# PANXIONG-CN/TEC-MoLLM

Hardware: AMD Instinct MI355X
Metric: train samples/sec (higher is better)
Workload: dtype f32; 1 GPU; BASELINE configs[1]: B=8/GPU, L_in=48, L_out=12, N=2911, F=10 (d_emb=12), 3 GPT-2 blocks, full fwd+bwd+AdamW, fp32, GATv2 per_timestep, dropout on (p=0.1); global_batch=8, parallelism=dp1, data_feed=fixed, launch=eager

## Files before the change

### include/tecmollm.h

```cpp
#ifndef TECMOLLM_H
#define TECMOLLM_H

#include <stdint.h>

#ifdef __cplusplus
extern "C" {
#endif

#define TECM_OK 0
#define TECM_E_ARG (-1)
#define TECM_E_ALIGN (-2)
#define TECM_E_LAUNCH (-3)
#define TECM_E_LDS (-4)

#define TECM_ABI_VERSION 21
int tecm_abi_version(void);
const char* tecm_last_error(void);

typedef struct TecmWin {
  int32_t enabled;
  int32_t N;
  int32_t Lin, Lout;
  int32_t stride_t;
  int32_t taps;
// ... 132 lines not shown
                       void* stream);

#define TECM_ATT_OUT_BF16 1
#define TECM_ATT_QKV_BF16 2
#define TECM_ATT_DCTX_BF16 4
int tecm_attention_fwd(const float* qkv, void* ctx, int32_t io_bf16, int32_t B, int32_t T, int32_t N, int32_t heads,
                       int32_t D, const TecmDrop* prob_drop, void* stream);
int tecm_attention_bwd(const float* qkv, const float* dctx, void* dqkv, int32_t io_bf16, int32_t B, int32_t T, int32_t N,
                       int32_t heads, int32_t D, const TecmDrop* prob_drop, void* stream);

int tecm_colsum(const float* in, int64_t ld, int64_t outer, int64_t inner, int32_t nseg, int32_t C,
                float* out, int64_t ldo, int32_t accumulate, float scale, const TecmDrop* in_drop,
                float* workspace , void* stream);
int tecm_colsum_twin(const float* in, int64_t ld, int64_t outer, int64_t inner, int32_t nseg, int32_t C,
                     float* out, int64_t ldo, int32_t accumulate, float scale, const TecmDrop* in_drop,
                     float* workspace, void* twin_bf16, int64_t ld_twin, void* stream);

int tecm_colsum_batch(const float* const* in, float* const* out, int32_t nbuf, int64_t ld, int64_t rows, int32_t C,
                      float* workspace , void* stream);

int tecm_huber_fwd_bwd(const float* pred, const float* target, float* dpred, float* loss_out,
                       int64_t n, float delta, float grad_scale, float* workspace ,
                       void* stream);

int tecm_conv_weight_pack(const float* w, float* fwd_pack, float* bwd_pack, int32_t Cout, int32_t Cin,
                          int32_t k, void* stream);
int tecm_conv_weight_unpack(const float* dpack, float* dw, int32_t Cout, int32_t Cin, int32_t k,
                            void* stream);

typedef struct TecmConvDx {
  const void* dy;
  const void* wpack;
  float* dinp;
  int32_t B, Lc, N, Cout, ld_in, _pad;
} TecmConvDx;
int tecm_conv_dx_pack(const float* w3, const float* w5, const float* w7, void* wpack, int32_t Cout, int32_t Cin,
                      int32_t ld_in, void* stream);
int tecm_conv_dx_bf16(const TecmConvDx* p, void* stream);
typedef struct TecmConvFwd {
  const void* inp;
  const void* wpack;
  const float* bias;
  float* y;
  int32_t B, Lc, N, Cout, ld_in, y_bf16;
  float* stats;
  float eps;
  int32_t _pad;
} TecmConvFwd;
int tecm_conv_fwd_pack(const float* w3, const float* w5, const float* w7, void* wpack, int32_t Cout, int32_t Cin,
                       int32_t ld_in, void* stream);
int tecm_conv_fwd_bf16(const TecmConvFwd* p, void* stream);
int tecm_conv_fwd_pack_f32(const float* w3, const float* w5, const float* w7, float* wpack, int32_t Cout, int32_t Cin,
                           int32_t ld_in, void* stream);
int tecm_conv_fwd_f32(const TecmConvFwd* p, void* stream);
int tecm_conv_dx_pack_f32(const float* w3, const float* w5, const float* w7, float* wpack, int32_t Cout, int32_t Cin,
                          int32_t ld_in, void* stream);
int tecm_conv_dx_f32(const TecmConvDx* p, void* stream);
int tecm_conv_fwd_supported(int32_t Lc, int32_t Cout, int32_t ld_in, int32_t f32);
int tecm_conv_dx_supported(int32_t Lc, int32_t Cout, int32_t ld_in, int32_t f32);
int tecm_conv_fwd_stats_supported(int32_t Lc);

typedef struct TecmConvDw {
  const void* inp;
  const void* dy;
  float* workspace;
  float* dw3;
  float* dw5;
// ... 103 lines not shown
```

### tec-mollm_amd/csrc/conv_seq.hip

```cpp
#include "common.h"
#include <type_traits>

typedef float f32x16 __attribute__((ext_vector_type(16)));
typedef __bf16 bf16x8 __attribute__((ext_vector_type(8)));
typedef unsigned int u32x4 __attribute__((ext_vector_type(4)));
typedef float f32x4 __attribute__((ext_vector_type(4)));

namespace tecm_convseq {

#ifndef CDX_ABLATE
#define CDX_ABLATE 0
#endif

constexpr int NB = 4;
constexpr int NTH = 256;
constexpr int MAXT = 6;

__host__ __device__ __forceinline__ int seg_nact(int d) {
  const int a = d < 3 ? 3 - d : d - 3;
  return a <= 1 ? 3 : (a == 2 ? 2 : 1);
}

struct Args {
  const void* dy;
// ... 129 lines not shown
#pragma unroll
        for (int gq = 0; gq < 4; ++gq) {
          const int ci = 32 * c + 8 * gq + 4 * h;
          if (ci < a.ld_in)
            *reinterpret_cast<float4*>(orow + ci) = make_float4(v[4 * gq], v[4 * gq + 1], v[4 * gq + 2], v[4 * gq + 3]);
        }
      }
    }
  }
}

template <int NCI>
__global__ __launch_bounds__(NTH, 2) void conv_dx_seq_kernel(const Args a) {
  extern __shared__ __attribute__((aligned(16))) unsigned char lds[];
  const int tid = threadIdx.x, lane = tid & 63;
  const int wave = __builtin_amdgcn_readfirstlane(tid >> 6);
  const Tile t = decode_tile(a, blockIdx.x);
  {
    constexpr int SB = 12;
    const int total = t.rows * a.cpr;
    for (int q0 = 0; q0 * NTH < ((CDX_ABLATE & 1) ? 0 : total); q0 += SB) {
      u32x4 v[SB];
      stage_load<SB>(a, t, q0, v);
      stage_store<SB>(a, t, q0, v, lds);
    }
    if (tid < a.pitch / 16) *reinterpret_cast<uint4*>(lds + a.zero_off + tid * 16) = make_uint4(0u, 0u, 0u, 0u);
  }
  __syncthreads();
  tile_compute<NCI>(a, t, lds, wave, lane, false);
}

constexpr int NTH32 = 512;

template <int NCI>
__global__ __launch_bounds__(NTH32, 2) void conv_dx_seq_f32_kernel(const Args a) {
  extern __shared__ __attribute__((aligned(16))) unsigned char lds[];
  const int tid = threadIdx.x, lane = tid & 63;
  const int wave = __builtin_amdgcn_readfirstlane(tid >> 6);
  const int r = lane & 31, h = lane >> 5;
  const Tile t = decode_tile(a, blockIdx.x);
  {
    constexpr int SB = 10;
    const int total = t.rows * a.cpr;
    for (int q0 = 0; q0 * NTH32 < total; q0 += SB) {
      u32x4 v[SB];
      stage_load<SB>(a, t, q0, v);
      stage_store<SB>(a, t, q0, v, lds);
    }
    if (tid < a.pitch / 16) *reinterpret_cast<uint4*>(lds + a.zero_off + tid * 16) = make_uint4(0u, 0u, 0u, 0u);
  }
  __syncthreads();

  const int spc = a.Cout / 8;
  const int KS = 15 * spc;
  const int s_beg = wave * (KS / 8), s_end = s_beg + KS / 8;
  int d = 0, sd = s_beg;
  while (sd >= seg_nact(d) * spc) {
    sd -= seg_nact(d) * spc;
    ++d;
  }
  const int ntt = t.tc >> 3;
  f32x16 acc[MAXT];
#pragma unroll
  for (int i = 0; i < MAXT; ++i)
#pragma unroll
    for (int e = 0; e < 16; ++e) acc[i][e] = 0.f;
  const int tl0 = r >> 2;
  constexpr int WD = 3;
  const f32x4* wp = reinterpret_cast<const f32x4*>(a.wpack) + (int64_t)s_beg * NCI * 64 + lane;
  f32x4 wf[WD][NCI];
#pragma unroll
  for (int u = 0; u < WD; ++u)
#pragma unroll
    for (int c = 0; c < NCI; ++c) wf[u][c] = wp[(u * NCI + c) * 64];
  for (int s0 = s_beg; s0 < s_end; s0 += WD) {
#pragma unroll
    for (int u = 0; u < WD; ++u) {
      const int delta = d - 3;
      const int colb = ((3 - seg_nact(d)) * a.Cout + sd * 8 + 4 * h) * 4;
      const int rbase = (t.t0 - t.ts_lo + delta) * 4 + r;
#pragma unroll
      for (int i = 0; i < MAXT / NCI; ++i) {
        if (i < ntt) {
          const int ts = t.t0 + 8 * i + tl0 + delta;
          const bool ok = ts >= 0 && ts < a.Lc;
          const int off = ok ? (rbase + 32 * i) * a.pitch + colb : a.zero_off + 16 * h;
          const f32x4 df = *reinterpret_cast<const f32x4*>(lds + off);
#pragma unroll
          for (int j = 0; j < 4; ++j)
#pragma unroll
            for (int c = 0; c < NCI; ++c)
              acc[i * NCI + c] = __builtin_amdgcn_mfma_f32_32x32x2f32(wf[u][c][j], df[j], acc[i * NCI + c], 0, 0, 0);
        }
      }
      if (s0 + u + WD < s_end) {
#pragma unroll
        for (int c = 0; c < NCI; ++c) wf[u][c] = wp[((u + WD) * NCI + c) * 64];
      }
      if (++sd == seg_nact(d) * spc) {
        sd = 0;
        ++d;
      }
    }
    wp += WD * NCI * 64;
  }
  __syncthreads();

  float* part = reinterpret_cast<float*>(lds);
  const int NT = ntt * NCI;
  if (wave >= 4) {
#pragma unroll
    for (int T = 0; T < MAXT; ++T)
      if (T < NT)
#pragma unroll
        for (int e = 0; e < 16; ++e) part[(((wave - 4) * NT + T) * 16 + e) * 64 + lane] = acc[T][e];
  }
  __syncthreads();
  if (wave < 4) {
#pragma unroll
    for (int T = 0; T < MAXT; ++T)
      if (T < NT)
#pragma unroll
        for (int e = 0; e < 16; ++e) acc[T][e] += part[((wave * NT + T) * 16 + e) * 64 + lane];
  }
  __syncthreads();
  if (wave < 4) {
#pragma unroll
    for (int T = 0; T < MAXT; ++T) {
      if (T < NT && (T & 3) != wave) {
        const int slot = (wave - (T & 3) - 1) & 3;
#pragma unroll
        for (int e = 0; e < 16; ++e) part[((T * 3 + slot) * 16 + e) * 64 + lane] = acc[T][e];
      }
    }
  }
  __syncthreads();
  if (wave < 4) {
#pragma unroll
    for (int T = 0; T < MAXT; ++T) {
      if (T < NT && (T & 3) == wave) {
        f32x16 v = acc[T];
#pragma unroll
        for (int slot = 0; slot < 3; ++slot)
#pragma unroll
          for (int e = 0; e < 16; ++e) v[e] += part[((T * 3 + slot) * 16 + e) * 64 + lane];
        const int i = T / NCI, c = T % NCI;
        const int tt = t.t0 + 8 * i + tl0, n = t.n0 + (r & 3);
        if (n < a.N) {
          float* orow = a.dinp + (((int64_t)t.b * a.Lc + tt) * a.N + n) * a.ld_in;
#pragma unroll
          for (int gq = 0; gq < 4; ++gq) {
            const int ci = 32 * c + 8 * gq + 4 * h;
            if (ci < a.ld_in)
              *reinterpret_cast<float4*>(orow + ci) = make_float4(v[4 * gq], v[4 * gq + 1], v[4 * gq + 2], v[4 * gq + 3]);
          }
        }
      }
    }
  }
}

__global__ __launch_bounds__(256) void conv_dx_pack_f32_kernel(const float* __restrict__ w3, const float* __restrict__ w5,
                                                               const float* __restrict__ w7, float* __restrict__ wpack,
                                                               int Cout, int Cin, int NCI) {
  const int total = 15 * Cout * NCI * 32;
  for (int i = blockIdx.x * 256 + threadIdx.x; i < total; i += gridDim.x * 256) {
    const int j = i & 3, lane = (i >> 2) & 63;
    const int sc = i >> 8, c = sc % NCI, s = sc / NCI;
    int k = 8 * s + 4 * (lane >> 5) + j;
    const int ci = 32 * c + (lane & 31);
    int d = 0;
    while (k >= seg_nact(d) * Cout) {
      k -= seg_nact(d) * Cout;
      ++d;
    }
    const int col = (3 - seg_nact(d)) * Cout + k;
    const int jj = col / Cout, co = col - jj * Cout;
    const int kj = 3 + 2 * jj, tau = (kj - 1) / 2 - (d - 3);
    const float* w = jj == 0 ? w3 : (jj == 1 ? w5 : w7);
    float v = 0.f;
    if (ci < Cin && tau >= 0 && tau < kj) v = w[((int64_t)co * Cin + ci) * kj + tau];
    wpack[i] = v;
  }
}

__global__ __launch_bounds__(256) void conv_dx_pack_kernel(const float* __restrict__ w3, const float* __restrict__ w5,
                                                           const float* __restrict__ w7, __bf16* __restrict__ wpack,
                                                           int Cout, int Cin, int NCI) {
  const int KTOT = 15 * Cout;
  const int total = KTOT * NCI * 32;
  for (int i = blockIdx.x * 256 + threadIdx.x; i < total; i += gridDim.x * 256) {
// ... 228 lines not shown
      if (i < ntt) {
#pragma unroll
        for (int e = 0; e < 16; ++e) {
          const int n = e & 3;
          if (n0 + n < a.N) yb[(8 * i + 2 * (e >> 2)) * tstride + n * CT] = acc[i][e] + bv;
        }
      }
    }
  }
  CFW_STAMP(8);
  if (a.stats) {
    __syncthreads();
    if (tid < 3 * NB) {
      const int jb = tid / NB, n = tid % NB;
      const float ucnt = (float)(32 * tc);
      float cnt = 0.f, mean = 0.f, m2 = 0.f;
      for (int w = 0; w < 4; ++w)
        for (int q = 0; q < 3; ++q)
          if (xst[w][q][0] == (float)jb) {
            const float tot = cnt + ucnt, fr = ucnt / tot, dl = xst[w][q][1 + n] - mean;
            m2 += xst[w][q][1 + NB + n] + dl * dl * cnt * fr;
            mean += dl * fr;
            cnt = tot;
          }
      if (n0 + n < a.N) {
        float* st = a.stats + (((int64_t)b * a.N + n0 + n) * 3 + jb) * 2;
        st[0] = mean;
        st[1] = 1.0f / sqrtf(m2 / cnt + a.eps);
      }
    }
  }
}

__global__ __launch_bounds__(NTH, 2) void conv_fwd_seq_f32_kernel(const FArgs a) {
  extern __shared__ __attribute__((aligned(16))) unsigned char lds[];
  const int tid = threadIdx.x, lane = tid & 63;
  const int wave = __builtin_amdgcn_readfirstlane(tid >> 6);
  const int r = lane & 31, h = lane >> 5;
  int tile = blockIdx.x;
  const int nbk = tile % a.nblk;
  tile /= a.nblk;
  const int chunk = tile % a.nchunk, b = tile / a.nchunk;
  const int n0 = nbk * NB, t0 = chunk * a.TC;
  const int tc = min(a.TC, a.Lc - t0);
  const int steps = tc + 7;
  const int CT = 3 * a.Cout;
  {
    const int cpr = a.ld_in / 4;
    const int total = steps * NB * cpr;
    const float* src = static_cast<const float*>(a.inp);
    for (int idx = tid; idx < total; idx += NTH) {
      const int row = idx / cpr, ch = idx - row * cpr;
      const int ts = t0 - 3 + (row >> 2);
      const int ng = min(n0 + (row & 3), a.N - 1);
      u32x4 v = {0u, 0u, 0u, 0u};
      if (ts >= 0 && ts < a.Lc)
        v = *reinterpret_cast<const u32x4*>(src + (((int64_t)b * a.Lc + ts) * a.N + ng) * a.ld_in + ch * 4);
      *reinterpret_cast<u32x4*>(lds + row * a.pitch + ch * 16) = v;
    }
  }
  __syncthreads();

  const int ntt = tc >> 3;
  const int cpt = a.ld_in / 4;
  const unsigned cpt_magic = (unsigned)((65536 + cpt - 1) / cpt);
#pragma unroll 1
  for (int ui = 0; ui < 3; ++ui) {
    const int u = (int)((a.assign >> (12 * wave + 4 * ui)) & 15ull);
    if (u == 15) break;
    const int j = u / a.nb32, kb = u - j * a.nb32;
    const int pad = j + 1, col0 = j * a.Cout + 32 * kb;
    const int st3 = 3 * a.ld_in / 8, st5 = 5 * a.ld_in / 8, st7 = 7 * a.ld_in / 8;
    const int nsteps = j == 0 ? st3 : (j == 1 ? st5 : st7);
    const int woff = (j == 0 ? 0 : (j == 1 ? st3 : st3 + st5)) * a.nb32 + kb * nsteps;
    f32x16 acc[MAXT];
#pragma unroll
    for (int i = 0; i < MAXT; ++i)
#pragma unroll
      for (int e = 0; e < 16; ++e) acc[i][e] = 0.f;
    const f32x4* wp = reinterpret_cast<const f32x4*>(a.wpack) + (int64_t)woff * 64 + lane;
    auto kloop = [&](auto ntc) {
      constexpr int NTT = decltype(ntc)::value;
      auto rd = [&](int s, f32x4 (&df)[NTT]) {
        const int q = 2 * s + h;
        const int tap = (int)((q * cpt_magic) >> 16), c4 = q - tap * cpt;
        const int off0 = ((tap - pad + 3) * 4 + r) * a.pitch + c4 * 16;
#pragma unroll
        for (int i = 0; i < NTT; ++i) df[i] = *reinterpret_cast<const f32x4*>(lds + off0 + 32 * i * a.pitch);
      };
      f32x4 wq[CFW_PD32], df[NTT];
#pragma unroll
      for (int p_ = 0; p_ < CFW_PD32; ++p_) wq[p_] = wp[min(p_, nsteps - 1) * 64];
      rd(0, df);
      for (int s = 0; s < nsteps; ++s) {
        const int sn = min(s + 1, nsteps - 1);
        const f32x4 wn = wp[min(s + CFW_PD32, nsteps - 1) * 64];
        f32x4 dn[NTT];
        rd(sn, dn);
#pragma unroll
        for (int jj = 0; jj < 4; ++jj)
#pragma unroll
          for (int i = 0; i < NTT; ++i) acc[i] = __builtin_amdgcn_mfma_f32_32x32x2f32(df[i][jj], wq[0][jj], acc[i], 0, 0, 0);
#pragma unroll
        for (int p_ = 0; p_ + 1 < CFW_PD32; ++p_) wq[p_] = wq[p_ + 1];
        wq[CFW_PD32 - 1] = wn;
#pragma unroll
        for (int i = 0; i < NTT; ++i) df[i] = dn[i];
      }
    };
    switch (ntt) {
      case 1: kloop(std::integral_constant<int, 1>{}); break;
      case 2: kloop(std::integral_constant<int, 2>{}); break;
      case 3: kloop(std::integral_constant<int, 3>{}); break;
      case 4: kloop(std::integral_constant<int, 4>{}); break;
      case 5: kloop(std::integral_constant<int, 5>{}); break;
      default: kloop(std::integral_constant<int, MAXT>{}); break;
    }
    const float bv = a.bias[col0 + r];
    float* yb = a.y + (((int64_t)b * a.Lc + t0 + h) * a.N + n0) * CT + col0 + r;
    const int tstride = a.N * CT;
#pragma unroll
    for (int i = 0; i < MAXT; ++i) {
      if (i < ntt) {
#pragma unroll
        for (int e = 0; e < 16; ++e) {
          const int n = e & 3;
          if (n0 + n < a.N) yb[(8 * i + 2 * (e >> 2)) * tstride + n * CT] = acc[i][e] + bv;
        }
      }
    }
  }
}

__global__ __launch_bounds__(256) void conv_fwd_pack_f32_kernel(const float* __restrict__ w3, const float* __restrict__ w5,
                                                                const float* __restrict__ w7, float* __restrict__ wpack,
                                                                int Cout, int Cin, int ld_in) {
  const int nblk = Cout / 32;
  int steps[3], base[3], tot = 0;
  for (int j = 0; j < 3; ++j) {
    steps[j] = (3 + 2 * j) * ld_in / 8;
    base[j] = tot;
    tot += steps[j] * nblk;
  }
  const int total = tot * 256;
  for (int i = blockIdx.x * 256 + threadIdx.x; i < total; i += gridDim.x * 256) {
    const int jj = i & 3, lane = (i >> 2) & 63, f = i >> 8;
    int j = 2;
    if (f < base[1]) j = 0; else if (f < base[2]) j = 1;
    const int fl = f - base[j], blk = fl / steps[j], s = fl - blk * steps[j];
    const int k = 8 * s + 4 * (lane >> 5) + jj;
    const int tap = k / ld_in, ci = k - tap * ld_in, kj = 3 + 2 * j;
    const float* w = j == 0 ? w3 : (j == 1 ? w5 : w7);
    float v = 0.f;
    if (tap < kj && ci < Cin) v = w[((int64_t)(32 * blk + (lane & 31)) * Cin + ci) * kj + tap];
    wpack[i] = v;
  }
}

__global__ __launch_bounds__(256) void conv_fwd_pack_kernel(const float* __restrict__ w3, const float* __restrict__ w5,
                                                            const float* __restrict__ w7, __bf16* __restrict__ wpack,
                                                            int Cout, int Cin, int ld_in) {
  const int nblk = Cout / 32;
  int steps[3], base[3], tot = 0;
// ... 133 lines not shown
  return TECM_OK;
}

struct ConvDxPlan { int TC, zero_off, row_bytes, pitch, NCI; size_t lds; };
static ConvDxPlan conv_dx_plan(int Lc, int Cout, int ld_in, bool f32) {
  using namespace tecm_convseq;
  ConvDxPlan q;
  q.NCI = (ld_in + 31) / 32;
  q.row_bytes = 3 * Cout * (f32 ? 4 : 2);
  q.pitch = q.row_bytes + 16;
  int TC = 8 * (MAXT / q.NCI);
  if (TC > Lc) TC = Lc;
  auto img_steps = [&](int tc) { return tc + 6 < Lc ? tc + 6 : Lc; };
  auto zero_of = [&](int tc) {
    const size_t img = (size_t)img_steps(tc) * NB * q.pitch;
    const size_t xch = (size_t)(tc / 8) * q.NCI * (f32 ? 4 : 3) * 16 * 64 * 4;
    return img > xch ? img : xch;
  };
  while (TC > 8 && zero_of(TC) + q.pitch > 160 * 1024) TC -= 8;
  q.TC = TC;
  q.zero_off = (int)zero_of(TC);
  q.lds = zero_of(TC) + q.pitch;
  return q;
}

extern "C" int tecm_conv_dx_supported(int32_t Lc, int32_t Cout, int32_t ld_in, int32_t f32) {
  if (Lc <= 0 || Lc % 8 != 0 || Cout <= 0 || Cout % 64 != 0 || ld_in <= 0 || ld_in % 4 != 0 || ld_in > 64) return 0;
  return conv_dx_plan(Lc, Cout, ld_in, f32 != 0).lds <= 160 * 1024 ? 1 : 0;
}

static int conv_dx_launch(const TecmConvDx* p, void* stream, bool f32, const char* who) {
  using namespace tecm_convseq;
  TECM_REQUIRE(p && p->dy && p->wpack && p->dinp, TECM_E_ARG, "%s: null pointer", who);
  TECM_REQUIRE(p->B > 0 && p->Lc > 0 && p->N > 0, TECM_E_ARG, "%s: bad shape", who);
  TECM_REQUIRE(p->Cout % 64 == 0 && p->Cout > 0 && p->ld_in % 4 == 0 && p->ld_in > 0 && p->ld_in <= 64, TECM_E_ARG,
               "%s: Cout must be a multiple of 64 and ld_in a multiple of 4 up to 64", who);
  TECM_REQUIRE(p->Lc % 8 == 0, TECM_E_ARG, "%s: the sequence length must be a multiple of 8", who);
  TECM_REQUIRE(tecm_aligned(p->dy, 16) && tecm_aligned(p->wpack, 16) && tecm_aligned(p->dinp, 16), TECM_E_ALIGN,
               "%s: 16-byte aligned pointers", who);
  Args a;
  a.dy = p->dy;
  a.wpack = p->wpack;
  a.dinp = p->dinp;
  a.B = p->B; a.Lc = p->Lc; a.N = p->N; a.Cout = p->Cout; a.ld_in = p->ld_in;
  const ConvDxPlan q = conv_dx_plan(p->Lc, p->Cout, p->ld_in, f32);
  a.NCI = q.NCI;
  a.row_bytes = q.row_bytes;
  a.cpr = a.row_bytes / 16;
  a.pitch = q.pitch;
  const size_t lds = q.lds;
  TECM_REQUIRE(lds <= 160 * 1024, TECM_E_LDS, "%s: %d channels need %zu B of LDS per tile", who, 3 * p->Cout, lds);
  const int TC = q.TC;
  a.TC = TC;
  a.zero_off = q.zero_off;
  a.nchunk = (p->Lc + TC - 1) / TC;
  a.nblk = (p->N + NB - 1) / NB;
  const int64_t tiles = (int64_t)p->B * a.nchunk * a.nblk;
  TECM_REQUIRE(tiles < ((int64_t)1 << 31), TECM_E_ARG, "%s: too many tiles", who);
  const void* fn = f32 ? (a.NCI == 1 ? reinterpret_cast<const void*>(&conv_dx_seq_f32_kernel<1>)
                                     : reinterpret_cast<const void*>(&conv_dx_seq_f32_kernel<2>))
                       : (a.NCI == 1 ? reinterpret_cast<const void*>(&conv_dx_seq_kernel<1>)
                                     : reinterpret_cast<const void*>(&conv_dx_seq_kernel<2>));
  TECM_REQUIRE(hipFuncSetAttribute(fn, hipFuncAttributeMaxDynamicSharedMemorySize, 160 * 1024) == hipSuccess, TECM_E_LAUNCH,
               "%s: hipFuncSetAttribute(MaxDynamicSharedMemorySize) failed", who);
  if (f32) {
    if (a.NCI == 1)
      hipLaunchKernelGGL(conv_dx_seq_f32_kernel<1>, dim3((unsigned)tiles), dim3(NTH32), lds, (hipStream_t)stream, a);
    else
      hipLaunchKernelGGL(conv_dx_seq_f32_kernel<2>, dim3((unsigned)tiles), dim3(NTH32), lds, (hipStream_t)stream, a);
  } else if (a.NCI == 1) {
    hipLaunchKernelGGL(conv_dx_seq_kernel<1>, dim3((unsigned)tiles), dim3(NTH), lds, (hipStream_t)stream, a);
  } else {
    hipLaunchKernelGGL(conv_dx_seq_kernel<2>, dim3((unsigned)tiles), dim3(NTH), lds, (hipStream_t)stream, a);
  }
  TECM_CHECK_LAUNCH("tecm_conv_dx");
  return TECM_OK;
}

extern "C" int tecm_conv_dx_bf16(const TecmConvDx* p, void* stream) { return conv_dx_launch(p, stream, false, "tecm_conv_dx_bf16"); }
extern "C" int tecm_conv_dx_f32(const TecmConvDx* p, void* stream) { return conv_dx_launch(p, stream, true, "tecm_conv_dx_f32"); }

extern "C" int tecm_conv_dx_pack_f32(const float* w3, const float* w5, const float* w7, float* wpack, int32_t Cout,
                                     int32_t Cin, int32_t ld_in, void* stream) {
  using namespace tecm_convseq;
  TECM_REQUIRE(w3 && w5 && w7 && wpack, TECM_E_ARG, "tecm_conv_dx_pack_f32: null pointer");
  TECM_REQUIRE(Cout > 0 && Cout % 64 == 0 && Cin > 0 && Cin <= ld_in && ld_in % 4 == 0, TECM_E_ARG,
               "tecm_conv_dx_pack_f32: Cout must be a multiple of 64, Cin <= ld_in, ld_in a multiple of 4");
  const int NCI = (ld_in + 31) / 32;
  const int total = 15 * Cout * NCI * 32;
  hipLaunchKernelGGL(conv_dx_pack_f32_kernel, dim3((total + 255) / 256), dim3(256), 0, (hipStream_t)stream, w3, w5, w7, wpack,
                     Cout, Cin, NCI);
  TECM_CHECK_LAUNCH("tecm_conv_dx_pack_f32");
  return TECM_OK;
}
```

### tec-mollm_amd/tecmollm/_lib.py

```python
from __future__ import annotations

import ctypes as C
import os
from typing import Optional

import torch

_HERE = os.path.dirname(os.path.abspath(__file__))
LIB_PATH = os.environ.get("TECM_LIB", os.path.join(_HERE, "libtecmollm_hip.so"))
ABI_VERSION = 21

c_f32p = C.c_void_p


class TecmWin(C.Structure):
    _fields_ = [("enabled", C.c_int32), ("N", C.c_int32), ("Lin", C.c_int32), ("Lout", C.c_int32),
                ("stride_t", C.c_int32), ("taps", C.c_int32), ("Cw", C.c_int32), ("pad", C.c_int32)]


class TecmDrop(C.Structure):
    _fields_ = [("p", C.c_float), ("_pad", C.c_int32), ("seed", C.c_uint64), ("ld", C.c_int64), ("seed_dev", C.c_void_p)]


class TecmGemm(C.Structure):
# ... 89 lines not shown

class TecmWindowBatch(C.Structure):
    _fields_ = [
        ("X", c_f32p), ("TF", c_f32p), ("Y", c_f32p), ("starts", C.c_void_p), ("starts_host_check", C.c_void_p),
        ("T", C.c_int64), ("row", C.c_int64),
        ("N", C.c_int32), ("L_in", C.c_int32), ("L_out", C.c_int32), ("F_t", C.c_int32), ("B", C.c_int32),
        ("_pad", C.c_int32),
        ("x_out", c_f32p), ("tf_out", c_f32p), ("y_out", c_f32p),
    ]


class TecmWindowBaseline(C.Structure):
    _fields_ = [
        ("X", c_f32p), ("starts", C.c_void_p), ("starts_host_check", C.c_void_p),
        ("T", C.c_int64),
        ("N", C.c_int32), ("C", C.c_int32), ("channel", C.c_int32), ("L_in", C.c_int32), ("L_out", C.c_int32),
        ("B", C.c_int32), ("mode", C.c_int32), ("period", C.c_int32),
        ("out", c_f32p), ("o_stride_b", C.c_int64), ("o_stride_h", C.c_int64), ("o_stride_n", C.c_int64),
    ]


class TecmSlotMean(C.Structure):
    _fields_ = [
        ("x", c_f32p), ("stride_t", C.c_int64), ("stride_n", C.c_int64),
        ("slot", C.c_void_p),
        ("T", C.c_int64), ("N", C.c_int32), ("n_slots", C.c_int32),
        ("means", C.c_void_p), ("counts", C.c_void_p),
    ]


class TecmConvDx(C.Structure):
    _fields_ = [("dy", C.c_void_p), ("wpack", C.c_void_p), ("dinp", c_f32p),
                ("B", C.c_int32), ("Lc", C.c_int32), ("N", C.c_int32), ("Cout", C.c_int32), ("ld_in", C.c_int32),
                ("_pad", C.c_int32)]


class TecmConvDw(C.Structure):
    _fields_ = [("inp", C.c_void_p), ("dy", C.c_void_p), ("workspace", c_f32p), ("dw3", c_f32p), ("dw5", c_f32p),
                ("dw7", c_f32p),
                ("B", C.c_int32), ("Lc", C.c_int32), ("N", C.c_int32), ("Cout", C.c_int32), ("Cin", C.c_int32),
                ("ld_in", C.c_int32), ("num_blocks", C.c_int32), ("_pad", C.c_int32)]


class TecmConvFwd(C.Structure):
    _fields_ = [("inp", C.c_void_p), ("wpack", C.c_void_p), ("bias", c_f32p), ("y", c_f32p),
                ("B", C.c_int32), ("Lc", C.c_int32), ("N", C.c_int32), ("Cout", C.c_int32), ("ld_in", C.c_int32),
                ("y_bf16", C.c_int32), ("stats", c_f32p), ("eps", C.c_float), ("_pad", C.c_int32)]


TECM_NORM_BLOCKS = 512
TECM_METRIC_STATS = 8
TECM_MAP_LDS_MAX_H = 32
TECM_BASELINE_MEAN, TECM_BASELINE_LAST, TECM_BASELINE_PERIODIC = 0, 1, 2


EXPORTS = {
    "tecm_abi_version": (C.c_int, []),
    "tecm_last_error": (C.c_char_p, []),
    "tecm_gemm_f32": (C.c_int, [C.POINTER(TecmGemm), C.c_void_p]),
    "tecm_gemm_bf16": (C.c_int, [C.POINTER(TecmGemm), C.c_void_p]),
    "tecm_gemm_bf16x3": (C.c_int, [C.POINTER(TecmGemm), C.c_void_p]),
    "tecm_gemm_bf16x6": (C.c_int, [C.POINTER(TecmGemm), C.c_void_p]),
    "tecm_gemm_last_kernel": (C.c_char_p, []),
    "tecm_spatial_fwd_lds_bytes": (C.c_int64, [C.c_int32, C.c_int32, C.c_int32]),
    "tecm_spatial_bwd_lds_bytes": (C.c_int64, [C.c_int32, C.c_int32, C.c_int32, C.c_int32]),
    "tecm_spatial_fwd": (C.c_int, [C.POINTER(TecmSpatial), C.c_void_p]),
    "tecm_spatial_fwd2_ws_floats": (C.c_int64, [C.POINTER(TecmSpatial)]),
# ... 118 lines not shown
```

### tec-mollm_amd/tecmollm/ops.py

```python
from __future__ import annotations

import os
import ctypes as C
from typing import List, Optional, Tuple

import torch

from . import _lib
from ._lib import TecmDrop, TecmGemm, TecmWin, check, lib, ptr, stream_ptr

A_MK, A_KM = 0, 1
B_NK, B_KN = 0, 1
ACT_NONE, ACT_GELU_ERF, ACT_GELU_TANH = 0, 1, 2

_MASK64 = (1 << 64) - 1


def splitmix64(x: int) -> int:
    x = (x + 0x9E3779B97F4A7C15) & _MASK64
    z = x
    z = ((z ^ (z >> 30)) * 0xBF58476D1CE4E5B9) & _MASK64
    z = ((z ^ (z >> 27)) * 0x94D049BB133111EB) & _MASK64
    return z ^ (z >> 31)

# ... 443 lines not shown
    vecs = [v.detach() for v in vecs]
    if any(v.dtype != torch.float32 or not v.is_contiguous() or v.dim() != 1 for v in vecs) or not 1 <= len(vecs) <= 12:
        raise _lib.TecmError("pack_vectors: 1..12 contiguous fp32 vectors")
    total = sum(v.numel() for v in vecs)
    if out is None:
        out = torch.empty(total, device=vecs[0].device, dtype=torch.float32)
    srcs = (C.c_void_p * len(vecs))(*[v.data_ptr() for v in vecs])
    lens = (C.c_int32 * len(vecs))(*[v.numel() for v in vecs])
    check(lib().tecm_pack_vectors(srcs, lens, len(vecs), out.data_ptr(), stream_ptr()), "tecm_pack_vectors")
    return out


def conv_weight_pack(w: torch.Tensor, want_bwd: bool = True) -> Tuple[torch.Tensor, Optional[torch.Tensor]]:
    Cout, Cin, k = w.shape
    fwd = torch.empty(Cout, k * Cin, device=w.device, dtype=torch.float32)
    bwd = torch.empty(k * Cout, Cin, device=w.device, dtype=torch.float32) if want_bwd else None
    check(lib().tecm_conv_weight_pack(w.data_ptr(), fwd.data_ptr(), ptr(bwd), Cout, Cin, k, stream_ptr()),
          "tecm_conv_weight_pack")
    return fwd, bwd


def conv_weight_unpack(dpack: torch.Tensor, Cout: int, Cin: int, k: int) -> torch.Tensor:
    dw = torch.empty(Cout, Cin, k, device=dpack.device, dtype=torch.float32)
    check(lib().tecm_conv_weight_unpack(dpack.data_ptr(), dw.data_ptr(), Cout, Cin, k, stream_ptr()),
          "tecm_conv_weight_unpack")
    return dw


def conv_dx_seq_ok(Lc: int, Cout: int, ld_in: int, f32: bool = False) -> bool:
    return (os.environ.get("TECM_CONV_SEQ", "1")[:1] != "0"
            and lib().tecm_conv_dx_supported(Lc, Cout, ld_in, 1 if f32 else 0) == 1)


def conv_dx(dy: torch.Tensor, w3: torch.Tensor, w5: torch.Tensor, w7: torch.Tensor, dinp: torch.Tensor, B: int,
            Lc: int, N: int, Cout: int, cin: int, ld_in: int) -> None:
    if dinp.dtype != torch.float32 or dy.dtype not in (torch.bfloat16, torch.float32):
        raise _lib.TecmError("conv_dx: dy is bf16 or fp32, dinp fp32")
    f32 = dy.dtype == torch.float32
    nci = (ld_in + 31) // 32
    wpack = torch.empty(15 * Cout * nci * 32, device=dy.device, dtype=dy.dtype)
    pack, run, what = ((lib().tecm_conv_dx_pack_f32, lib().tecm_conv_dx_f32, "tecm_conv_dx_f32") if f32 else
                       (lib().tecm_conv_dx_pack, lib().tecm_conv_dx_bf16, "tecm_conv_dx_bf16"))
    check(pack(w3.data_ptr(), w5.data_ptr(), w7.data_ptr(), wpack.data_ptr(), Cout, cin, ld_in, stream_ptr()), what + "/pack")
    d = _lib.TecmConvDx(dy=dy.data_ptr(), wpack=wpack.data_ptr(), dinp=dinp.data_ptr(), B=B, Lc=Lc, N=N, Cout=Cout,
                        ld_in=ld_in)
    if _timing is None:
        check(run(C.byref(d), stream_ptr()), what)
        return
    e0, e1 = torch.cuda.Event(enable_timing=True), torch.cuda.Event(enable_timing=True)
    e0.record()
    check(run(C.byref(d), stream_ptr()), what)
    e1.record()
    name = ("conv_dx_seq_f32_kernel" if f32 else "conv_dx_seq_kernel") + \
        (f" M={B * Lc * N} N={ld_in} K={15 * Cout}" if _timing_detail else "")
    _timing.append((name, 2.0 * B * Lc * N * ld_in * 15 * Cout, e0, e1))


conv_dx_bf16 = conv_dx


def conv_dw_seq_ok(Lc: int, Cout: int, ld_in: int) -> bool:
    return os.environ.get("TECM_CONV_DW_SEQ", "1")[:1] != "0" and lib().tecm_conv_dw_supported(Lc, Cout, ld_in) == 1


_cu_count = {}


def conv_dw(inp: torch.Tensor, dy: torch.Tensor, B: int, Lc: int, N: int, Cout: int, cin: int, ld_in: int):
    if inp.dtype != dy.dtype or dy.dtype not in (torch.bfloat16, torch.float32):
        raise _lib.TecmError("conv_dw: inp and dy are both bf16 or both fp32 tensors")
    f32 = dy.dtype == torch.float32
    run, what = (lib().tecm_conv_dw_f32, "tecm_conv_dw_f32") if f32 else (lib().tecm_conv_dw_bf16, "tecm_conv_dw_bf16")
    dev = dy.device
    nb = _cu_count.get(dev.index)
    if nb is None:
        nb = _cu_count[dev.index] = int(os.environ.get("TECM_CONV_DW_BLOCKS", 0)) or \
            torch.cuda.get_device_properties(dev).multi_processor_count
    nws = lib().tecm_conv_dw_workspace(Cout, ld_in, nb)
# ... 66 lines not shown
```

Baseline: 124.8 samples/s.

## Add persistent pipelined fp32 conv dx kernel that prefetches the next tile during compute

Adds a persistent fp32 conv dx kernel with a grid sized to the CU count. Each block loops over tiles and issues global loads for the next tile's input into registers while the MFMA loop for the current tile runs. The K loop is also specialized on the row-tile count, so LDS reads for all row tiles are batched ahead of the MFMAs. This aims to hide global-to-LDS staging latency and per-block launch overhead, at the cost of extra prefetch registers that may reduce occupancy. Optional timestamp instrumentation is included but compiled out by default.

```diff
diff --git a/include/tecmollm.h b/include/tecmollm.h
--- a/include/tecmollm.h
+++ b/include/tecmollm.h
@@ -188,7 +188,8 @@
   const void* dy;
   const void* wpack;
   float* dinp;
-  int32_t B, Lc, N, Cout, ld_in, _pad;
+  int32_t B, Lc, N, Cout, ld_in;
+  int32_t num_blocks;
 } TecmConvDx;
 int tecm_conv_dx_pack(const float* w3, const float* w5, const float* w7, void* wpack, int32_t Cout, int32_t Cin,
                       int32_t ld_in, void* stream);
diff --git a/tec-mollm_amd/csrc/conv_seq.hip b/tec-mollm_amd/csrc/conv_seq.hip
--- a/tec-mollm_amd/csrc/conv_seq.hip
+++ b/tec-mollm_amd/csrc/conv_seq.hip
@@ -185,25 +185,22 @@
 
 constexpr int NTH32 = 512;
 
-template <int NCI>
-__global__ __launch_bounds__(NTH32, 2) void conv_dx_seq_f32_kernel(const Args a) {
-  extern __shared__ __attribute__((aligned(16))) unsigned char lds[];
-  const int tid = threadIdx.x, lane = tid & 63;
-  const int wave = __builtin_amdgcn_readfirstlane(tid >> 6);
+#ifdef CSQ32_STAMPS
+__device__ unsigned long long csq32_stamps[8 * 8192];
+}
+extern "C" int tecm_csq32_stamps_read(unsigned long long* dst, int n) {
+  return (int)hipMemcpyFromSymbol(dst, HIP_SYMBOL(tecm_convseq::csq32_stamps), sizeof(unsigned long long) * n);
+}
+namespace tecm_convseq {
+#define CSQ32_STAMP(slot, i) do { if (threadIdx.x == 0 && (slot) < 8192) csq32_stamps[(slot) * 8 + (i)] = __builtin_amdgcn_s_memrealtime(); } while (0)
+#else
+#define CSQ32_STAMP(slot, i) do { } while (0)
+#endif
+
+template <int NCI, int PF>
+__device__ __forceinline__ void dx32_tile(const Args& a, const Tile& t, const Tile& tn, u32x4 (&pf)[PF > 0 ? PF : 1],
+                                          unsigned char* lds, int wave, int lane, int slot) {
   const int r = lane & 31, h = lane >> 5;
-  const Tile t = decode_tile(a, blockIdx.x);
-  {
-    constexpr int SB = 10;
-    const int total = t.rows * a.cpr;
-    for (int q0 = 0; q0 * NTH32 < total; q0 += SB) {
-      u32x4 v[SB];
-      stage_load<SB>(a, t, q0, v);
-      stage_store<SB>(a, t, q0, v, lds);
-    }
-    if (tid < a.pitch / 16) *reinterpret_cast<uint4*>(lds + a.zero_off + tid * 16) = make_uint4(0u, 0u, 0u, 0u);
-  }
-  __syncthreads();
-
   const int spc = a.Cout / 8;
   const int KS = 15 * spc;
   const int s_beg = wave * (KS / 8), s_end = s_beg + KS / 8;
@@ -226,41 +223,64 @@
   for (int u = 0; u < WD; ++u)
 #pragma unroll
     for (int c = 0; c < NCI; ++c) wf[u][c] = wp[(u * NCI + c) * 64];
-  for (int s0 = s_beg; s0 < s_end; s0 += WD) {
-#pragma unroll
-    for (int u = 0; u < WD; ++u) {
-      const int delta = d - 3;
-      const int colb = ((3 - seg_nact(d)) * a.Cout + sd * 8 + 4 * h) * 4;
-      const int rbase = (t.t0 - t.ts_lo + delta) * 4 + r;
-#pragma unroll
-      for (int i = 0; i < MAXT / NCI; ++i) {
-        if (i < ntt) {
+  if constexpr (PF > 0) stage_load<PF>(a, tn, 0, pf);
+  CSQ32_STAMP(slot, 2);
+  auto kloop = [&](auto ntc) {
+    constexpr int NTT = decltype(ntc)::value;
+    for (int s0 = s_beg; s0 < ((CDX_ABLATE & 2) ? s_beg : s_end); s0 += WD) {
+#pragma unroll
+      for (int u = 0; u < WD; ++u) {
+        const int delta = d - 3;
+        const int colb = ((3 - seg_nact(d)) * a.Cout + sd * 8 + 4 * h) * 4;
+        const int rbase = (t.t0 - t.ts_lo + delta) * 4 + r;
+        f32x4 df[NTT];
+#pragma unroll
+        for (int i = 0; i < NTT; ++i) {
           const int ts = t.t0 + 8 * i + tl0 + delta;
           const bool ok = ts >= 0 && ts < a.Lc;
           const int off = ok ? (rbase + 32 * i) * a.pitch + colb : a.zero_off + 16 * h;
-          const f32x4 df = *reinterpret_cast<const f32x4*>(lds + off);
-#pragma unroll
-          for (int j = 0; j < 4; ++j)
+          df[i] = *reinterpret_cast<const f32x4*>(lds + off);
+        }
+#pragma unroll
+        for (int j = 0; j < 4; ++j)
+#pragma unroll
+          for (int i = 0; i < NTT; ++i)
 #pragma unroll
             for (int c = 0; c < NCI; ++c)
-              acc[i * NCI + c] = __builtin_amdgcn_mfma_f32_32x32x2f32(wf[u][c][j], df[j], acc[i * NCI + c], 0, 0, 0);
+              acc[i * NCI + c] = __builtin_amdgcn_mfma_f32_32x32x2f32(wf[u][c][j], df[i][j], acc[i * NCI + c], 0, 0, 0);
+        const int ahead = s0 + u + WD < s_end ? WD : 0;
+#pragma unroll
+        for (int c = 0; c < NCI; ++c) wf[u][c] = wp[((u + ahead) * NCI + c) * 64];
+        if (++sd == seg_nact(d) * spc) {
+          sd = 0;
+          ++d;
         }
       }
-      if (s0 + u + WD < s_end) {
-#pragma unroll
-        for (int c = 0; c < NCI; ++c) wf[u][c] = wp[((u + WD) * NCI + c) * 64];
-      }
-      if (++sd == seg_nact(d) * spc) {
-        sd = 0;
-        ++d;
-      }
-    }
-    wp += WD * NCI * 64;
-  }
+      wp += WD * NCI * 64;
+    }
+  };
+  static_assert(MAXT == 6 && (NCI == 1 || NCI == 2), "row tiles per wave");
+  if constexpr (NCI == 1) {
+    switch (ntt) {
+      case 1: kloop(std::integral_constant<int, 1>{}); break;
+      case 2: kloop(std::integral_constant<int, 2>{}); break;
+      case 3: kloop(std::integral_constant<int, 3>{}); break;
+      case 4: kloop(std::integral_constant<int, 4>{}); break;
+      case 5: kloop(std::integral_constant<int, 5>{}); break;
+      default: kloop(std::integral_constant<int, 6>{}); break;
+    }
+  } else {
+    switch (ntt) {
+      case 1: kloop(std::integral_constant<int, 1>{}); break;
+      case 2: kloop(std::integral_constant<int, 2>{}); break;
+      default: kloop(std::integral_constant<int, 3>{}); break;
+    }
+  }
+  CSQ32_STAMP(slot, 3);
   __syncthreads();
 
   float* part = reinterpret_cast<float*>(lds);
-  const int NT = ntt * NCI;
+  const int NT = (CDX_ABLATE & 4) ? 0 : ntt * NCI;
   if (wave >= 4) {
 #pragma unroll
     for (int T = 0; T < MAXT; ++T)
@@ -291,12 +311,13 @@
   if (wave < 4) {
 #pragma unroll
     for (int T = 0; T < MAXT; ++T) {
-      if (T < NT && (T & 3) == wave) {
+      if (T < ntt * NCI && (T & 3) == wave) {
         f32x16 v = acc[T];
 #pragma unroll
-        for (int slot = 0; slot < 3; ++slot)
-#pragma unroll
-          for (int e = 0; e < 16; ++e) v[e] += part[((T * 3 + slot) * 16 + e) * 64 + lane];
+        for (int sl = 0; sl < ((CDX_ABLATE & 4) ? 0 : 3); ++sl)
+#pragma unroll
+          for (int e = 0; e < 16; ++e) v[e] += part[((T * 3 + sl) * 16 + e) * 64 + lane];
+        if (T < 4) CSQ32_STAMP(slot, 4);
         const int i = T / NCI, c = T % NCI;
         const int tt = t.t0 + 8 * i + tl0, n = t.n0 + (r & 3);
         if (n < a.N) {
@@ -310,6 +331,63 @@
         }
       }
     }
+  }
+  CSQ32_STAMP(slot, 5);
+}
+
+template <int NCI>
+__global__ __launch_bounds__(NTH32, 2) void conv_dx_seq_f32_kernel(const Args a) {
+  extern __shared__ __attribute__((aligned(16))) unsigned char lds[];
+  CSQ32_STAMP(blockIdx.x, 0);
+  const int tid = threadIdx.x, lane = tid & 63;
+  const int wave = __builtin_amdgcn_readfirstlane(tid >> 6);
+  const Tile t = decode_tile(a, blockIdx.x);
+  {
+    constexpr int SB = 10;
+    const int total = t.rows * a.cpr;
+    for (int q0 = 0; q0 * NTH32 < ((CDX_ABLATE & 1) ? 0 : total); q0 += SB) {
+      u32x4 v[SB];
+      stage_load<SB>(a, t, q0, v);
+      stage_store<SB>(a, t, q0, v, lds);
+    }
+    if (tid < a.pitch / 16) *reinterpret_cast<uint4*>(lds + a.zero_off + tid * 16) = make_uint4(0u, 0u, 0u, 0u);
+  }
+  __syncthreads();
+  CSQ32_STAMP(blockIdx.x, 1);
+  u32x4 none[1];
+  dx32_tile<NCI, 0>(a, t, t, none, lds, wave, lane, blockIdx.x);
+}
+
+#ifndef DX32_PF
+#define DX32_PF (NCI == 1 ? 12 : 10)
+#endif
+template <int NCI>
+__global__ __launch_bounds__(NTH32, 2) void conv_dx_seq_f32_pipe_kernel(const Args a, const int tiles) {
+  extern __shared__ __attribute__((aligned(16))) unsigned char lds[];
+  constexpr int PF = DX32_PF, SB = 2;
+  const int tid = threadIdx.x, lane = tid & 63;
+  const int wave = __builtin_amdgcn_readfirstlane(tid >> 6);
+  int tile = blockIdx.x;
+  CSQ32_STAMP(tile, 0);
+  Tile t = decode_tile(a, tile);
+  u32x4 pf[PF];
+  stage_load<PF>(a, t, 0, pf);
+  if (tid < a.pitch / 16) *reinterpret_cast<uint4*>(lds + a.zero_off + tid * 16) = make_uint4(0u, 0u, 0u, 0u);
+  for (; tile < tiles; tile += gridDim.x) {
+    if (!(CDX_ABLATE & 1)) stage_store<PF>(a, t, 0, pf, lds);
+    for (int q0 = PF; q0 * NTH32 < ((CDX_ABLATE & 1) ? 0 : t.rows * a.cpr); q0 += SB) {
+      u32x4 v[SB];
+      stage_load<SB>(a, t, q0, v);
+      stage_store<SB>(a, t, q0, v, lds);
+    }
+    __syncthreads();
+    CSQ32_STAMP(tile, 1);
+    const int next = tile + (int)gridDim.x;
+    const Tile tn = decode_tile(a, next < tiles ? next : tile);
+    dx32_tile<NCI, PF>(a, t, tn, pf, lds, wave, lane, tile);
+    __syncthreads();
+    CSQ32_STAMP(next, 0);
+    t = tn;
   }
 }
 
@@ -604,11 +682,81 @@
   }
 }
 
+__device__ __forceinline__ void fwd32_unit(const FArgs& a, const unsigned char* lds, const int u, const int b, const int n0,
+                                           const int t0, const int tc, const int lane) {
+  const int r = lane & 31, h = lane >> 5;
+  const int CT = 3 * a.Cout;
+  const int ntt = tc >> 3;
+  const int cpt = a.ld_in / 4;
+  const unsigned cpt_magic = (unsigned)((65536 + cpt - 1) / cpt);
+  const int j = u / a.nb32, kb = u - j * a.nb32;
+  const int pad = j + 1, col0 = j * a.Cout + 32 * kb;
+  const int st3 = 3 * a.ld_in / 8, st5 = 5 * a.ld_in / 8, st7 = 7 * a.ld_in / 8;
+  const int nsteps = j == 0 ? st3 : (j == 1 ? st5 : st7);
+  const int woff = (j == 0 ? 0 : (j == 1 ? st3 : st3 + st5)) * a.nb32 + kb * nsteps;
+  f32x16 acc[MAXT];
+#pragma unroll
+  for (int i = 0; i < MAXT; ++i)
+#pragma unroll
+    for (int e = 0; e < 16; ++e) acc[i][e] = 0.f;
+  const f32x4* wp = reinterpret_cast<const f32x4*>(a.wpack) + (int64_t)woff * 64 + lane;
+  auto kloop = [&](auto ntc) {
+    constexpr int NTT = decltype(ntc)::value;
+    auto rd = [&](int s, f32x4 (&df)[NTT]) {
+      const int q = 2 * s + h;
+      const int tap = (int)((q * cpt_magic) >> 16), c4 = q - tap * cpt;
+      const int off0 = ((tap - pad + 3) * 4 + r) * a.pitch + c4 * 16;
+#pragma unroll
+      for (int i = 0; i < NTT; ++i) df[i] = *reinterpret_cast<const f32x4*>(lds + off0 + 32 * i * a.pitch);
+    };
+    f32x4 wq[CFW_PD32], df[NTT];
+#pragma unroll
+    for (int p_ = 0; p_ < CFW_PD32; ++p_) wq[p_] = wp[min(p_, nsteps - 1) * 64];
+    rd(0, df);
+    for (int s = 0; s < nsteps; ++s) {
+      const int sn = min(s + 1, nsteps - 1);
+      const f32x4 wn = wp[min(s + CFW_PD32, nsteps - 1) * 64];
+      f32x4 dn[NTT];
+      rd(sn, dn);
+#pragma unroll
+      for (int jj = 0; jj < 4; ++jj)
+#pragma unroll
+        for (int i = 0; i < NTT; ++i) acc[i] = __builtin_amdgcn_mfma_f32_32x32x2f32(df[i][jj], wq[0][jj], acc[i], 0, 0, 0);
+#pragma unroll
+      for (int p_ = 0; p_ + 1 < CFW_PD32; ++p_) wq[p_] = wq[p_ + 1];
+      wq[CFW_PD32 - 1] = wn;
+#pragma unroll
+      for (int i = 0; i < NTT; ++i) df[i] = dn[i];
+    }
+  };
+  switch (ntt) {
+    case 1: kloop(std::integral_constant<int, 1>{}); break;
+    case 2: kloop(std::integral_constant<int, 2>{}); break;
+    case 3: kloop(std::integral_constant<int, 3>{}); break;
+    case 4: kloop(std::integral_constant<int, 4>{}); break;
+    case 5: kloop(std::integral_constant<int, 5>{}); break;
+    default: kloop(std::integral_constant<int, MAXT>{}); break;
+  }
+  const float bv = a.bias[col0 + r];
+  float* yb = a.y + (((int64_t)b * a.Lc + t0 + h) * a.N + n0) * CT + col0 + r;
+  const int tstride = a.N * CT;
+#pragma unroll
+  for (int i = 0; i < MAXT; ++i) {
+    if (i < ntt) {
+#pragma unroll
+      for (int e = 0; e < 16; ++e) {
+        const int n = e & 3;
+        if (n0 + n < a.N) yb[(8 * i + 2 * (e >> 2)) * tstride + n * CT] = acc[i][e] + bv;
+      }
+    }
+  }
+}
+
 __global__ __launch_bounds__(NTH, 2) void conv_fwd_seq_f32_kernel(const FArgs a) {
   extern __shared__ __attribute__((aligned(16))) unsigned char lds[];
+  CSQ32_STAMP(blockIdx.x, 0);
   const int tid = threadIdx.x, lane = tid & 63;
   const int wave = __builtin_amdgcn_readfirstlane(tid >> 6);
-  const int r = lane & 31, h = lane >> 5;
   int tile = blockIdx.x;
   const int nbk = tile % a.nblk;
   tile /= a.nblk;
@@ -616,7 +764,6 @@
   const int n0 = nbk * NB, t0 = chunk * a.TC;
   const int tc = min(a.TC, a.Lc - t0);
   const int steps = tc + 7;
-  const int CT = 3 * a.Cout;
   {
     const int cpr = a.ld_in / 4;
     const int total = steps * NB * cpr;
@@ -632,75 +779,13 @@
     }
   }
   __syncthreads();
-
-  const int ntt = tc >> 3;
-  const int cpt = a.ld_in / 4;
-  const unsigned cpt_magic = (unsigned)((65536 + cpt - 1) / cpt);
+  CSQ32_STAMP(blockIdx.x, 1);
 #pragma unroll 1
   for (int ui = 0; ui < 3; ++ui) {
     const int u = (int)((a.assign >> (12 * wave + 4 * ui)) & 15ull);
     if (u == 15) break;
-    const int j = u / a.nb32, kb = u - j * a.nb32;
-    const int pad = j + 1, col0 = j * a.Cout + 32 * kb;
-    const int st3 = 3 * a.ld_in / 8, st5 = 5 * a.ld_in / 8, st7 = 7 * a.ld_in / 8;
-    const int nsteps = j == 0 ? st3 : (j == 1 ? st5 : st7);
-    const int woff = (j == 0 ? 0 : (j == 1 ? st3 : st3 + st5)) * a.nb32 + kb * nsteps;
-    f32x16 acc[MAXT];
-#pragma unroll
-    for (int i = 0; i < MAXT; ++i)
-#pragma unroll
-      for (int e = 0; e < 16; ++e) acc[i][e] = 0.f;
-    const f32x4* wp = reinterpret_cast<const f32x4*>(a.wpack) + (int64_t)woff * 64 + lane;
-    auto kloop = [&](auto ntc) {
-      constexpr int NTT = decltype(ntc)::value;
-      auto rd = [&](int s, f32x4 (&df)[NTT]) {
-        const int q = 2 * s + h;
-        const int tap = (int)((q * cpt_magic) >> 16), c4 = q - tap * cpt;
-        const int off0 = ((tap - pad + 3) * 4 + r) * a.pitch + c4 * 16;
-#pragma unroll
-        for (int i = 0; i < NTT; ++i) df[i] = *reinterpret_cast<const f32x4*>(lds + off0 + 32 * i * a.pitch);
-      };
-      f32x4 wq[CFW_PD32], df[NTT];
-#pragma unroll
-      for (int p_ = 0; p_ < CFW_PD32; ++p_) wq[p_] = wp[min(p_, nsteps - 1) * 64];
-      rd(0, df);
-      for (int s = 0; s < nsteps; ++s) {
-        const int sn = min(s + 1, nsteps - 1);
-        const f32x4 wn = wp[min(s + CFW_PD32, nsteps - 1) * 64];
-        f32x4 dn[NTT];
-        rd(sn, dn);
-#pragma unroll
-        for (int jj = 0; jj < 4; ++jj)
-#pragma unroll
-          for (int i = 0; i < NTT; ++i) acc[i] = __builtin_amdgcn_mfma_f32_32x32x2f32(df[i][jj], wq[0][jj], acc[i], 0, 0, 0);
-#pragma unroll
-        for (int p_ = 0; p_ + 1 < CFW_PD32; ++p_) wq[p_] = wq[p_ + 1];
-        wq[CFW_PD32 - 1] = wn;
-#pragma unroll
-        for (int i = 0; i < NTT; ++i) df[i] = dn[i];
-      }
-    };
-    switch (ntt) {
-      case 1: kloop(std::integral_constant<int, 1>{}); break;
-      case 2: kloop(std::integral_constant<int, 2>{}); break;
-      case 3: kloop(std::integral_constant<int, 3>{}); break;
-      case 4: kloop(std::integral_constant<int, 4>{}); break;
-      case 5: kloop(std::integral_constant<int, 5>{}); break;
-      default: kloop(std::integral_constant<int, MAXT>{}); break;
-    }
-    const float bv = a.bias[col0 + r];
-    float* yb = a.y + (((int64_t)b * a.Lc + t0 + h) * a.N + n0) * CT + col0 + r;
-    const int tstride = a.N * CT;
-#pragma unroll
-    for (int i = 0; i < MAXT; ++i) {
-      if (i < ntt) {
-#pragma unroll
-        for (int e = 0; e < 16; ++e) {
-          const int n = e & 3;
-          if (n0 + n < a.N) yb[(8 * i + 2 * (e >> 2)) * tstride + n * CT] = acc[i][e] + bv;
-        }
-      }
-    }
+    fwd32_unit(a, lds, u, b, n0, t0, tc, lane);
+    CSQ32_STAMP(blockIdx.x, 3 + ui);
   }
 }
 
@@ -900,7 +985,7 @@
 static int conv_dx_launch(const TecmConvDx* p, void* stream, bool f32, const char* who) {
   using namespace tecm_convseq;
   TECM_REQUIRE(p && p->dy && p->wpack && p->dinp, TECM_E_ARG, "%s: null pointer", who);
-  TECM_REQUIRE(p->B > 0 && p->Lc > 0 && p->N > 0, TECM_E_ARG, "%s: bad shape", who);
+  TECM_REQUIRE(p->B > 0 && p->Lc > 0 && p->N > 0 && p->num_blocks >= 0, TECM_E_ARG, "%s: bad shape", who);
   TECM_REQUIRE(p->Cout % 64 == 0 && p->Cout > 0 && p->ld_in % 4 == 0 && p->ld_in > 0 && p->ld_in <= 64, TECM_E_ARG,
                "%s: Cout must be a multiple of 64 and ld_in a multiple of 4 up to 64", who);
   TECM_REQUIRE(p->Lc % 8 == 0, TECM_E_ARG, "%s: the sequence length must be a multiple of 8", who);
@@ -925,13 +1010,23 @@
   a.nblk = (p->N + NB - 1) / NB;
   const int64_t tiles = (int64_t)p->B * a.nchunk * a.nblk;
   TECM_REQUIRE(tiles < ((int64_t)1 << 31), TECM_E_ARG, "%s: too many tiles", who);
-  const void* fn = f32 ? (a.NCI == 1 ? reinterpret_cast<const void*>(&conv_dx_seq_f32_kernel<1>)
+  const bool pipe = f32 && p->num_blocks > 0;
+  const void* fn = pipe ? (a.NCI == 1 ? reinterpret_cast<const void*>(&conv_dx_seq_f32_pipe_kernel<1>)
+                                      : reinterpret_cast<const void*>(&conv_dx_seq_f32_pipe_kernel<2>))
+                   : f32 ? (a.NCI == 1 ? reinterpret_cast<const void*>(&conv_dx_seq_f32_kernel<1>)
                                      : reinterpret_cast<const void*>(&conv_dx_seq_f32_kernel<2>))
                        : (a.NCI == 1 ? reinterpret_cast<const void*>(&conv_dx_seq_kernel<1>)
                                      : reinterpret_cast<const void*>(&conv_dx_seq_kernel<2>));
   TECM_REQUIRE(hipFuncSetAttribute(fn, hipFuncAttributeMaxDynamicSharedMemorySize, 160 * 1024) == hipSuccess, TECM_E_LAUNCH,
                "%s: hipFuncSetAttribute(MaxDynamicSharedMemorySize) failed", who);
-  if (f32) {
+  if (pipe) {
+    const unsigned grid = (unsigned)(tiles < p->num_blocks ? tiles : p->num_blocks);
+    TECM_REQUIRE(tiles + p->num_blocks < ((int64_t)1 << 31), TECM_E_ARG, "%s: too many tiles", who);
+    if (a.NCI == 1)
+      hipLaunchKernelGGL(conv_dx_seq_f32_pipe_kernel<1>, dim3(grid), dim3(NTH32), lds, (hipStream_t)stream, a, (int)tiles);
+    else
+      hipLaunchKernelGGL(conv_dx_seq_f32_pipe_kernel<2>, dim3(grid), dim3(NTH32), lds, (hipStream_t)stream, a, (int)tiles);
+  } else if (f32) {
     if (a.NCI == 1)
       hipLaunchKernelGGL(conv_dx_seq_f32_kernel<1>, dim3((unsigned)tiles), dim3(NTH32), lds, (hipStream_t)stream, a);
     else
diff --git a/tec-mollm_amd/tecmollm/_lib.py b/tec-mollm_amd/tecmollm/_lib.py
--- a/tec-mollm_amd/tecmollm/_lib.py
+++ b/tec-mollm_amd/tecmollm/_lib.py
@@ -145,7 +145,7 @@
 class TecmConvDx(C.Structure):
     _fields_ = [("dy", C.c_void_p), ("wpack", C.c_void_p), ("dinp", c_f32p),
                 ("B", C.c_int32), ("Lc", C.c_int32), ("N", C.c_int32), ("Cout", C.c_int32), ("ld_in", C.c_int32),
-                ("_pad", C.c_int32)]
+                ("num_blocks", C.c_int32)]
 
 
 class TecmConvDw(C.Structure):
diff --git a/tec-mollm_amd/tecmollm/ops.py b/tec-mollm_amd/tecmollm/ops.py
--- a/tec-mollm_amd/tecmollm/ops.py
+++ b/tec-mollm_amd/tecmollm/ops.py
@@ -499,6 +499,19 @@
             and lib().tecm_conv_dx_supported(Lc, Cout, ld_in, 1 if f32 else 0) == 1)
 
 
+_conv_seq_blocks = {}
+
+
+def _conv_dx_grid(dev) -> int:
+    if os.environ.get("TECM_CONV_DX_PIPE", "1")[:1] == "0":
+        return 0
+    nb = _conv_seq_blocks.get(dev.index)
+    if nb is None:
+        nb = _conv_seq_blocks[dev.index] = int(os.environ.get("TECM_CONV_SEQ_BLOCKS", 0)) or \
+            torch.cuda.get_device_properties(dev).multi_processor_count
+    return nb
+
+
 def conv_dx(dy: torch.Tensor, w3: torch.Tensor, w5: torch.Tensor, w7: torch.Tensor, dinp: torch.Tensor, B: int,
             Lc: int, N: int, Cout: int, cin: int, ld_in: int) -> None:
     if dinp.dtype != torch.float32 or dy.dtype not in (torch.bfloat16, torch.float32):
@@ -510,7 +523,7 @@
                        (lib().tecm_conv_dx_pack, lib().tecm_conv_dx_bf16, "tecm_conv_dx_bf16"))
     check(pack(w3.data_ptr(), w5.data_ptr(), w7.data_ptr(), wpack.data_ptr(), Cout, cin, ld_in, stream_ptr()), what + "/pack")
     d = _lib.TecmConvDx(dy=dy.data_ptr(), wpack=wpack.data_ptr(), dinp=dinp.data_ptr(), B=B, Lc=Lc, N=N, Cout=Cout,
-                        ld_in=ld_in)
+                        ld_in=ld_in, num_blocks=_conv_dx_grid(dy.device) if f32 else 0)
     if _timing is None:
         check(run(C.byref(d), stream_ptr()), what)
         return
```

New measurement: 125.2 samples/s, median of 6. About the same (+0.3%).
